# soulslicer/probabilistic-depth

Measured on AMD Instinct MI355X. Metric: depth-volumes/sec (D=64, 256x512), higher is better.
Workload: dtype f32 (fp16-pair products on MFMA, fp32 accumulate)

## Files before the change

### probabilistic-depth_amd/csrc/sweep_dist.hip

```cpp
#include <hip/hip_runtime.h>

#include <atomic>
#include <climits>
#include <cstdlib>

#include "dist_layout.hpp"
#include "epipolar_probe.hpp"
#include "geometry.hpp"
#include "kernels.hpp"
#include "sweep_workspace.hpp"
#include "wave_util.hpp"

#include "sweep_dist_knobs.hpp"

namespace pdepth {

namespace {

using namespace wv;
typedef _Float16 h8 __attribute__((ext_vector_type(8)));
typedef _Float16 h2 __attribute__((ext_vector_type(2)));
typedef int v2i __attribute__((ext_vector_type(2)));

constexpr int DIST_MAXV = 8;

struct DistArgs {
    SweepArgs a;
    const char* packed;
    const float* stats;
    int* queue;
    int* qcnt;
    int qstride;
    int tiles_x, ntile;
    int one_each;
    int nblk;
    int nonce;
};
#define KARG(type, field) kernarg_at<type>(offsetof(DistArgs, field))


__device__ __forceinline__ float dist_exp(float x) {
    return __builtin_amdgcn_exp2f((x < -1000.0f ? -1000.0f : x) * 1.44269502162933349609375f);
}

template <int MAXB, int NAC>
struct __attribute__((aligned(16))) DistLds {
    static constexpr int XSTRIDE = MAXB * 16 + 4;
    float Ys[16 * XSTRIDE];
    float Qs[(MAXB + 3) / 4 * 256 + 8];
    _Float16 Bs[NAC * 4 * 16 * 8];
    float rp[4 * 16 * 2];
    float mus[dist::MAX_C + 8];
    float xf[DIST_MAXV * 12];
    float cst[8];
    float red[4 * 16 * 4];
    float dcl[128];
    int ctab[2][64 * 2];
    int ired[2][2];
    int brow[MAXB + 2];
    v4i rec[2];
    int iflag;
    unsigned char wide[64];
};

template <int NCHK, int NH>
__global__ __launch_bounds__(256, NH == 1 ? DIST_OCC1 : DIST_OCC2) void sweep_dist_kernel(DistArgs da) {
    constexpr int NAC = 2 * NCHK + 1;
    constexpr int MP = NCHK + 1;
    constexpr int MAXB = NH == 1 ? DIST_MAXB1 : DIST_MAXB2;
    constexpr int NC = 4 * NH;
    constexpr int QPL = 8 * NCHK + 3;
    constexpr int NS = NH == 1 ? DIST_SETS1 : DIST_SETS2;
    typedef DistLds<MAXB, NAC> Lds;
    constexpr int XSTRIDE = Lds::XSTRIDE;
    __shared__ Lds L;
#ifdef DIST_STAMPS
    unsigned long long stamp_acc[12] = {0, 0, 0, 0, 0, 0, 0, 0, 0, 0, 0, 0};
    unsigned long long stamp_t = __builtin_amdgcn_s_memtime();
#endif
    if (poison_on_foreign_layout(da.a, da.queue, LAYOUT_DIST16)) return;
    const int tid = threadIdx.x;

    {
        const float* dc = KARG(const float*, a.d_candi);
        const int D = KARG(int, a.D);
        for (int k = tid; k < 64 * NH; k += 256) L.dcl[k] = dc[min(k, D - 1)];
    }
    if (tid < 128) { L.ctab[0][tid] = (tid & 1) ? INT_MIN : INT_MAX; L.ctab[1][tid] = (tid & 1) ? INT_MIN : INT_MAX; }
    if (tid < 64) L.wide[tid] = 1;
    if (tid < 2) { L.ired[tid][0] = INT_MAX; L.ired[tid][1] = INT_MIN; }
    __syncthreads();
    if ((int)(tid >> 2) < min(KARG(int, a.B), 64) && epipolar_probe_is_steep(da.a, tid >> 2, tid & 3)) L.wide[tid >> 2] = 0;

    const int xcd = blockIdx.x & 7;
    if (blockIdx.x == 0 && tid == 0) KARG(int*, queue)[DIST_NONCE_SLOT] = KARG(int, nonce);
    auto band_tiles_of = [&](int q) { const int nt = KARG(int, ntile); return (nt >> 3) + (q < (nt & 7) ? 1 : 0); };
    auto band_first_of = [&](int q) {
        const int nt = KARG(int, ntile), qq = nt >> 3, rr8 = nt & 7;
        return q < rr8 ? q * (qq + 1) : rr8 * (qq + 1) + (q - rr8) * qq;
    };
    auto items_of = [&](int q) { return 4 * band_tiles_of(q) * KARG(int, a.B); };
    int own_done = 0;
    auto steal = [&]() -> int {
        int* qcnt = KARG(int*, qcnt);
        const int qs = KARG(int, qstride);
#pragma unroll 1
        for (int j = 1; j < 8; ++j) {
            const int q = (opaque_s(xcd) + j) & 7, nq = items_of(q);
            if (__hip_atomic_load(&qcnt[q * qs], __ATOMIC_RELAXED, __HIP_MEMORY_SCOPE_AGENT) >= nq) continue;
            const int got = atomicAdd(&qcnt[q * qs], 1);
            if (got < nq) return (q << 28) | got;
        }
        return -1;
    };
    auto resolve = [&](int got) -> int {
        const int n_own = items_of(xcd);
        if (!own_done && got < n_own) return (opaque_s(xcd) << 28) | got;
        own_done = 1;
        return steal();
    };
    auto fdiv = [](int nn, int dd) { return (int)(((float)nn + 0.5f) * __builtin_amdgcn_rcpf((float)dd)); };
    auto decode = [&](int item, int& b_, int& tx_, int& ty_, int& sub_) {
        const int ntile = KARG(int, ntile), tiles_x = KARG(int, tiles_x), H = KARG(int, a.H);
        const int qq = ntile >> 3, rr8 = ntile & 7;
        const bool small_idx = (long long)ntile * 4 * KARG(int, a.B) < (1ll << 22);
        const int tiles_y_ = (H + 3) / 4;
        const int q_ = item >> 28, iq = item & 0x0fffffff, band_tiles = band_tiles_of(q_);
        const int tidx = iq >> 2;
        sub_ = iq & 3;
        b_ = small_idx ? fdiv(tidx, band_tiles) : tidx / band_tiles;
        const int ti = tidx - b_ * band_tiles;
        int tile = band_first_of(q_) + ti;
        if (rr8 == 0 && tiles_y_ % 16 == 0 && tiles_y_ * tiles_x == ntile) {
            const int hb_rows = tiles_y_ / 16, half_tiles = hb_rows * tiles_x;
            const int second = ti >= half_tiles ? 1 : 0, tih = ti - second * half_tiles;
            const int hbi = (q_ < 4) == (second == 0) ? q_ : 8 + q_;
            const int cc = small_idx ? fdiv(tih, hb_rows) : tih / hb_rows, r_ = tih - cc * hb_rows;
            tile = (hbi * hb_rows + r_) * tiles_x + cc;
        } else if (rr8 == 0 && qq % tiles_x == 0) {
            const int band_rows = qq / tiles_x, tc = small_idx ? fdiv(ti, band_rows) : ti / band_rows;
            tile = (q_ * band_rows + (ti - tc * band_rows)) * tiles_x + tc;
        }
        ty_ = small_idx ? fdiv(tile, tiles_x) : tile / tiles_x;
        tx_ = tile - ty_ * tiles_x;
    };
#define ONE_EACH (KARG(int, one_each) != 0)
    __syncthreads();

    int state = 0;
    int n_direct = 0;
    int got_own = (tid == 0 && !ONE_EACH) ? atomicAdd(&KARG(int*, qcnt)[xcd * KARG(int, qstride)], 1) : (int)(blockIdx.x >> 3);
    int next_item = -1;
    auto resolve_next = [&]() { if (opaque_v((int)threadIdx.x) == 0) next_item = ONE_EACH ? -1 : resolve(got_own); };
    constexpr int REC_WIDE = 1, REC_BELOW = 2, REC_FIRST = 4;
    auto publish = [&](int slot, int item) {
        v4i r = v4i{item, 0, 0, 0};
        if (item >= 0) {
            int b, tx, ty, sub;
            decode(item, b, tx, ty, sub);
            const bool wide = b < 64 ? L.wide[b] != 0 : false;
            const int x0 = wide ? tx * 16 : tx * 16 + 8 * (sub & 1), y0 = wide ? ty * 4 + sub : ty * 4 + 2 * (sub >> 1);
            r.y = b;
            r.z = (y0 << 16) | x0;
            r.w = (wide ? REC_WIDE : 0) | (y0 >= KARG(int, a.H) ? REC_BELOW : 0) | ((tx | ty | sub) == 0 ? REC_FIRST : 0);
        }
        L.rec[slot] = r;
    };
    constexpr bool EARLY = DIST_DECODE_EARLY != 0;
    constexpr bool POP_EARLY = EARLY && DIST_PREFETCH == 0;
    auto record_next = [&]() {
        if (opaque_v((int)threadIdx.x) == 0) {
            publish(state & 1, next_item);
            if (POP_EARLY && !ONE_EACH && !own_done) got_own = atomicAdd(&KARG(int*, qcnt)[xcd * KARG(int, qstride)], 1);
        }
    };
    auto publish_next = [&]() {
        if (opaque_v((int)threadIdx.x) == 0) {
            if (!EARLY) publish(state & 1, next_item);
            if (!POP_EARLY && !ONE_EACH && !own_done) got_own = atomicAdd(&KARG(int*, qcnt)[xcd * KARG(int, qstride)], 1);
        }
    };
    constexpr bool PF = DIST_PREFETCH != 0;
    constexpr int ZW = 64 + 128 * NCHK;
    static_assert(4 * ZW + 128 <= (int)(sizeof(Lds::Qs) / sizeof(float)), "the prefetch zone does not fit L.Qs");
    auto dma_pixels = [&](int wave, int b, int p4) {
        const int H = KARG(int, a.H), W = KARG(int, a.W), C = KARG(int, a.C), HW = H * W;
        const int kq = (opaque_v((int)threadIdx.x) & 63) >> 4;
        const __amdgpu_buffer_rsrc_t rray =
            __builtin_amdgcn_make_buffer_rsrc((void*)(KARG(const float*, a.rays) + (size_t)b * 3 * HW), 0, 3 * HW * 4, 0x00020000);
        const __amdgpu_buffer_rsrc_t rref = __builtin_amdgcn_make_buffer_rsrc(
            (void*)(KARG(const float*, a.ref) + (size_t)b * KARG(long long, a.ref_bstride)), 0, C * HW * 4, 0x00020000);
        dma_b32(rray, lds_addr_of(&L.Qs[wave * ZW]), kq < 3 ? kq * HW * 4 + p4 : OOB, 0);
#pragma unroll
        for (int mm = 0; mm < NCHK; ++mm)
#pragma unroll
            for (int j = 0; j < 2; ++j) {
                const int cr = 8 * wave + 4 * j + kq;
                dma_b32(rref, lds_addr_of(&L.Qs[wave * ZW + 64 + 128 * mm + 64 * j]), cr < C - 32 * mm ? cr * HW * 4 + p4 : OOB, 32 * mm * HW * 4);
            }
        if (wave == 0) {
#pragma unroll
            for (int j = 0; j < 2; ++j) {
                const int cr = 4 * j + kq;
                dma_b32(rref, lds_addr_of(&L.Qs[4 * ZW + 64 * j]), cr < C - 32 * NCHK ? cr * HW * 4 + p4 : OOB, 32 * NCHK * HW * 4);
            }
        }
    };
    auto prefetch_next = [&](int wave) {
        const v4i nrec = L.rec[state & 1];
        if (__builtin_amdgcn_readfirstlane(nrec.x) < 0) return;
        const int fl = __builtin_amdgcn_readfirstlane(nrec.w);
        if (fl & REC_BELOW) return;
        const int b = __builtin_amdgcn_readfirstlane(nrec.y), xy = __builtin_amdgcn_readfirstlane(nrec.z);
        const int H = KARG(int, a.H), W = KARG(int, a.W);
        const int n = opaque_v((int)threadIdx.x) & 15;
        const int x = (xy & 0xffff) + ((fl & REC_WIDE) ? n : (n & 7));
        const int y = (xy >> 16) + ((fl & REC_WIDE) ? 0 : (n >> 3));
        dma_pixels(wave, b, (min(y, H - 1) * W + min(x, W - 1)) * 4);
        state |= 4;
    };
    if (tid == 0) {
        publish(0, ONE_EACH ? (got_own < items_of(xcd) ? (xcd << 28) | got_own : -1) : resolve(got_own));
        if (!ONE_EACH && !own_done) got_own = atomicAdd(&KARG(int*, qcnt)[xcd * KARG(int, qstride)], 1);
    }
    PDEPTH_LDS_BARRIER();
#define PDEPTH_POP_WAIT(n) __builtin_amdgcn_s_waitcnt(0x0f70 | (n))
    PDEPTH_POP_WAIT(0);

    for (;;) {
        const v4i rec = L.rec[state & 1];
        state ^= 1;
        const int pf = state & 4;
        state ^= pf;
        if (__builtin_amdgcn_readfirstlane(rec.x) < 0) break;
        DSTAMP(0)
        const int wave = opaque_s(__builtin_amdgcn_readfirstlane((int)threadIdx.x >> 6));
        const int b = __builtin_amdgcn_readfirstlane(rec.y), xy0 = __builtin_amdgcn_readfirstlane(rec.z), recfl = __builtin_amdgcn_readfirstlane(rec.w);
        const int H = KARG(int, a.H), W = KARG(int, a.W), V = KARG(int, a.V), C = KARG(int, a.C), D = KARG(int, a.D);
        const bool wide = (recfl & REC_WIDE) != 0;

        {
            if (recfl & REC_BELOW) {
                resolve_next();
                if (EARLY) record_next();
                publish_next();
                PDEPTH_LDS_BARRIER();
                PDEPTH_POP_WAIT(0);
                continue;
            }
            const int tid = opaque_v((int)threadIdx.x), lane = tid & 63;
            const int n = lane & 15, kq = lane >> 4, tq = wave * 4 + kq;
            const int a32 = (lane ^ 32) << 2;
            const int HW = H * W;
            int p;
            bool xlive;
            float ray[3], rv[MP][2];
            {
                const __amdgpu_buffer_rsrc_t rray =
                    __builtin_amdgcn_make_buffer_rsrc((void*)(KARG(const float*, a.rays) + (size_t)b * 3 * HW), 0, 3 * HW * 4, 0x00020000);
                const __amdgpu_buffer_rsrc_t rref = __builtin_amdgcn_make_buffer_rsrc(
                    (void*)(KARG(const float*, a.ref) + (size_t)b * KARG(long long, a.ref_bstride)), 0, C * HW * 4, 0x00020000);
                const int x = (xy0 & 0xffff) + (wide ? n : (n & 7));
                const int y = (xy0 >> 16) + (wide ? 0 : (n >> 3));
                xlive = x < W && y < H;
                p = min(y, H - 1) * W + min(x, W - 1);
                if (PF) {
                    if (!pf) dma_pixels(wave, b, p * 4);
                } else {
#pragma unroll
                    for (int i = 0; i < 3; ++i) ray[i] = __builtin_bit_cast(float, __builtin_amdgcn_raw_buffer_load_b32(rray, p * 4, i * HW * 4, 0));
#pragma unroll
                    for (int mm = 0; mm < MP; ++mm) {
                        const bool mine = mm < NCHK || wave == 0;
#pragma unroll
                        for (int i = 0; i < 2; ++i)
                            rv[mm][i] = __builtin_bit_cast(float, __builtin_amdgcn_raw_buffer_load_b32(
                                rref, mine && 2 * tq + i < C - 32 * mm ? ((2 * tq + i) * HW + p) * 4 : OOB, 32 * mm * HW * 4, 0));
                    }
                }
            }
            if (EARLY) { resolve_next(); record_next(); }
            DSTAMP(1)
            const bool new_b = b + 1 != state >> 3;
            if (new_b) {
                state = (state & 7) | ((b + 1) << 3);
                const int tid = opaque_v((int)threadIdx.x), lane = tid & 63;
                const float* st = KARG(const float*, stats) + (size_t)b * STATS_STRIDE;
                if (wave == 0) {
                    float am = st[STATS_AMAX + lane], sv = st[STATS_VAR + lane], sl_ = st[STATS_LAG + lane], m2 = st[lane] * st[lane];
                    if (lane + 64 < STATS_VAR) {
                        am = fmaxf(am, st[STATS_AMAX + lane + 64]); sv += st[STATS_VAR + lane + 64]; sl_ += st[STATS_LAG + lane + 64];
                        m2 += st[lane + 64] * st[lane + 64];
                    }
                    float dhi = fabsf(L.dcl[lane]), dlo = -dhi;
                    if (NH == 2) { const float d2 = fabsf(L.dcl[lane + 64]); dhi = fmaxf(dhi, d2); dlo = fmaxf(dlo, -d2); }
                    {
                        const int x32 = (lane ^ 32) << 2;
                        am = fmaxf(am, bperm_f(x32, am)); sv += bperm_f(x32, sv); sl_ += bperm_f(x32, sl_); m2 += bperm_f(x32, m2);
                        dhi = fmaxf(dhi, bperm_f(x32, dhi)); dlo = fmaxf(dlo, bperm_f(x32, dlo));
#define PDEPTH_XOR_STEP(M) { const int pat = ((M) << 10) | 0x1f; \
                             am = fmaxf(am, __builtin_bit_cast(float, __builtin_amdgcn_ds_swizzle(__builtin_bit_cast(int, am), pat))); \
                             sv += __builtin_bit_cast(float, __builtin_amdgcn_ds_swizzle(__builtin_bit_cast(int, sv), pat)); \
                             sl_ += __builtin_bit_cast(float, __builtin_amdgcn_ds_swizzle(__builtin_bit_cast(int, sl_), pat)); \
                             m2 += __builtin_bit_cast(float, __builtin_amdgcn_ds_swizzle(__builtin_bit_cast(int, m2), pat)); \
                             dhi = fmaxf(dhi, __builtin_bit_cast(float, __builtin_amdgcn_ds_swizzle(__builtin_bit_cast(int, dhi), pat))); \
                             dlo = fmaxf(dlo, __builtin_bit_cast(float, __builtin_amdgcn_ds_swizzle(__builtin_bit_cast(int, dlo), pat))); }
                        PDEPTH_XOR_STEP(16) PDEPTH_XOR_STEP(8) PDEPTH_XOR_STEP(4) PDEPTH_XOR_STEP(2) PDEPTH_XOR_STEP(1)
#undef PDEPTH_XOR_STEP
                    }
                    const int e = dist::scale_exponent(am);
                    const float sc = ldexpf(1.0f, e);
                    const float sg = KARG(float, a.sigma);
                    const bool outside = sv > DIST_GUARD_RATIO * sl_ && sv * 10.0f > DIST_GUARD_ENERGY * fabsf(sg);
                    const bool illcond = (float)KARG(int, a.V) * (2.0f * sv + m2) * (dhi + dlo) * 1.1920929e-7f > PDEPTH_COND_LIMIT * fabsf(sg);
                    if (lane == 0) {
                        L.cst[6] = sc; L.cst[7] = ldexpf(refined_rcp(sg), -2 * e);
                        const int pf = reinterpret_cast<const int*>(st + STATS_FLAGS)[0];
                        L.iflag = (pf != 0 ? 1 : 0) | (outside ? 2 : 0) | (illcond ? 4 : 0);
                    }
                    for (int c = lane; c < dist::MAX_C + 8; c += 64) L.mus[c] = st[c] * sc;
                }
                if (tid >= 128 && tid < 128 + V) {
                    const int v = tid - 128;
                    ViewXform xf;
                    make_view_xform(KARG(const float*, a.K) + b * 9, KARG(const float*, a.R) + ((size_t)b * V + v) * 9,
                                    KARG(const float*, a.t) + ((size_t)b * V + v) * 3, KARG(int, a.blas_mode), xf);
    #pragma unroll
                    for (int i = 0; i < 9; ++i) L.xf[v * 12 + i] = xf.kr[i];
    #pragma unroll
                    for (int i = 0; i < 3; ++i) L.xf[v * 12 + 9 + i] = xf.kt[i];
                }
                if (tid == 255) {
                    const float* const cxcy_ = KARG(const float*, a.cxcy);
                    const float cx = cxcy_[b * 2 + 0], cy = cxcy_[b * 2 + 1];
                    L.cst[0] = cx; L.cst[1] = cy; L.cst[2] = refined_rcp(cx); L.cst[3] = refined_rcp(cy);
                    L.cst[4] = (float)W / 2.0f; L.cst[5] = (float)H / 2.0f;
                }
            }
            bool item_ready = !new_b;
            if (KARG(const float*, a.src) != nullptr) {
                if (!item_ready) { PDEPTH_LDS_BARRIER(); item_ready = true; }
                if ((__builtin_amdgcn_readfirstlane(L.iflag) & 7) != 0) {
                    if (opaque_v((int)threadIdx.x) == 0 && (recfl & REC_FIRST)) {
                        reinterpret_cast<int*>(const_cast<float*>(KARG(const float*, stats)) + (size_t)b * STATS_STRIDE + STATS_FLAGS)[1] = 1;
                        n_direct += KARG(int, tiles_x) * (wide ? H : 2 * ((H + 1) >> 1));
                    }
                    if (!EARLY) resolve_next();
                    publish_next();
                    PDEPTH_LDS_BARRIER();
                    PDEPTH_POP_WAIT(0);
                    continue;
                }
            }
            float rr = 0.0f, zc = 0.0f;
            bool centred = false;
            unsigned failmask = 0;
            float cost[NC];
#pragma unroll
            for (int j = 0; j < NC; ++j) cost[j] = 0.0f;
            if (PF) {
                if (pf && (KARG(float*, a.logp_out) != nullptr || KARG(float*, a.depth_out) != nullptr)) {
                    if (NC == 4) asm volatile("s_waitcnt vmcnt(4)" ::: "memory");
                    else asm volatile("s_waitcnt vmcnt(8)" ::: "memory");
                } else {
                    asm volatile("s_waitcnt vmcnt(0)" ::: "memory");
                }
                const float* const z = &L.Qs[wave * ZW];
#pragma unroll
                for (int i = 0; i < 3; ++i) ray[i] = z[16 * i + n];
#pragma unroll
                for (int mm = 0; mm < MP; ++mm)
#pragma unroll
                    for (int i = 0; i < 2; ++i)
                        rv[mm][i] = mm < NCHK ? z[64 + 128 * mm + 16 * (2 * kq + i) + n] : (wave == 0 ? L.Qs[4 * ZW + 16 * (2 * kq + i) + n] : 0.0f);
            }

            constexpr bool RETRY = NH == 2;
            for (int v = 0; v < V; ++v) {
                const char* const srcv_v = RETRY ? nullptr : KARG(const char*, packed) + (size_t)((size_t)b * V + v) * dist::view_bytes(C, H, W);
                const int H_ = H, W_ = W, C_ = C, D_ = D;
#pragma unroll
                for (int h = 0; h < NH; ++h) {
                    if (!item_ready) { PDEPTH_LDS_BARRIER(); item_ready = true; }
                    int attempt = 0;
                    for (;;) {
                    const bool mine = attempt == 0 || (wave >> 1) == attempt - 1;
                    const int H = RETRY ? KARG(int, a.H) : H_, W = RETRY ? KARG(int, a.W) : W_, C = RETRY ? KARG(int, a.C) : C_, D = RETRY ? KARG(int, a.D) : D_;
                    int cell[4];
                    float fw[4], fn[4];
                    {
                        ViewXform xf;
                        {
                            const v4f k0 = *reinterpret_cast<const v4f*>(&L.xf[v * 12]), k1 = *reinterpret_cast<const v4f*>(&L.xf[v * 12 + 4]),
                                      k2 = *reinterpret_cast<const v4f*>(&L.xf[v * 12 + 8]);
                            xf.kr[0] = k0.x; xf.kr[1] = k0.y; xf.kr[2] = k0.z; xf.kr[3] = k0.w; xf.kr[4] = k1.x; xf.kr[5] = k1.y;
                            xf.kr[6] = k1.z; xf.kr[7] = k1.w; xf.kr[8] = k2.x; xf.kt[0] = k2.y; xf.kt[1] = k2.z; xf.kt[2] = k2.w;
                            xf.separate = KARG(int, a.blas_mode);
                        }
                        const v4f c0 = *reinterpret_cast<const v4f*>(&L.cst[0]);
                        const v2f c1 = *reinterpret_cast<const v2f*>(&L.cst[4]);
                        const v4f dk = *reinterpret_cast<const v4f*>(&L.dcl[64 * h + 4 * tq]);
                        float t2a, t2b, t2c;
                        ray_term2(xf, ray[0], ray[1], ray[2], t2a, t2b, t2c);
#pragma unroll
                        for (int j = 0; j < 4; ++j) {
                            const int k = 64 * h + 4 * tq + j;
                            float ix, iy;
                            plane_sample_pos_fast(xf, t2a, t2b, t2c, dk[j], c0.x, c0.y, c0.z, c0.w, c1.x, c1.y, ix, iy);
                            cell[j] = cell_of(ix, iy, W, H, fw[j], fn[j]);
                            if (k >= D || !xlive || !mine) cell[j] = NO_CELL;
                        }
#pragma unroll
                        for (int j = 0; j < 4; ++j) { asm volatile("" : "+v"(fw[j])); asm volatile("" : "+v"(fn[j])); }
                    }
                    DSTAMP(2)
                    if (!centred) {
                        const float sc = L.cst[6], sm2 = -2.0f * sc;
                        float pr = 0.0f, pz = 0.0f;
                        int* const Bw = reinterpret_cast<int*>(L.Bs);
#pragma unroll
                        for (int mm = 0; mm < MP; ++mm) {
                            if (mm == NCHK && wave != 0) continue;
                            const v2f mu2 = *reinterpret_cast<const v2f*>(&L.mus[32 * mm + 2 * tq]);
                            const float x0 = __builtin_fmaf(rv[mm][0], sm2, 2.0f * mu2.x), x1 = __builtin_fmaf(rv[mm][1], sm2, 2.0f * mu2.y);
                            const float s0 = rv[mm][0] * sc, s1 = rv[mm][1] * sc;
                            pr = __builtin_fmaf(x0, x0, pr); pr = __builtin_fmaf(x1, x1, pr);
                            pz = __builtin_fmaf(s0, s0, pz); pz = __builtin_fmaf(s1, s1, pz);
                            const h2 bh = __builtin_convertvector(v2f{x0, x1}, h2);
                            const h2 bl = __builtin_convertvector(v2f{x0 - (float)bh.x, x1 - (float)bh.y}, h2);
                            if (mm < NCHK) {
                                Bw[((mm * 4 + wave) * 16 + n) * 4 + kq] = __builtin_bit_cast(int, bh);
                                Bw[(((NCHK + mm) * 4 + wave) * 16 + n) * 4 + kq] = __builtin_bit_cast(int, bl);
                            } else {
                                Bw[(((2 * NCHK) * 4 + 0) * 16 + n) * 4 + kq] = __builtin_bit_cast(int, bh);
                                Bw[(((2 * NCHK) * 4 + 1) * 16 + n) * 4 + kq] = __builtin_bit_cast(int, bh);
                                Bw[(((2 * NCHK) * 4 + 2) * 16 + n) * 4 + kq] = __builtin_bit_cast(int, bl);
                            }
                        }
                        pr = 0.25f * pr;
                        pr = pr + xor16_f(pr); pr = pr + bperm_f(a32, pr);
                        pz = pz + xor16_f(pz); pz = pz + bperm_f(a32, pz);
                        if (kq == 0) *reinterpret_cast<v2f*>(&L.rp[(wave * 16 + n) * 2]) = v2f{pr, pz};
                    }
                    const int par = (state >> 1) & 1;
                    {
                        int ylo = 32767, yhi = -32768;
                        int rmin = 0, rmax = 0, ry = 0;
                        bool open = false;
#pragma unroll
                        for (int j = 0; j < 4; ++j) {
                            const bool vj = cell[j] != NO_CELL;
                            const int yj = cell_y(cell[j]), xj = cell_x(cell[j]);
                            const bool cont = open && vj && yj == ry;
                            if (open && !cont) {
                                atomicMin(&L.ctab[par][(ry & 63) * 2], rmin);
                                atomicMax(&L.ctab[par][(ry & 63) * 2 + 1], rmax);
                            }
                            rmin = cont ? min(rmin, xj) : xj;
                            rmax = cont ? max(rmax, xj) : xj;
                            ry = yj;
                            open = vj;
                            ylo = min(ylo, vj ? yj : 32767);
                            yhi = max(yhi, yj);
                        }
                        if (open) {
                            atomicMin(&L.ctab[par][(ry & 63) * 2], rmin);
                            atomicMax(&L.ctab[par][(ry & 63) * 2 + 1], rmax);
                        }
                        const int wmin = wave_min_i(ylo), wmax = wave_max_i(yhi);
                        if (lane == 0 && wmin <= wmax) { atomicMin(&L.ired[par][0], wmin); atomicMax(&L.ired[par][1], wmax); }
                    }
                    DSTAMP(3)
                    PDEPTH_LDS_BARRIER();
                    DSTAMP(4)
                    if (!centred) {
#pragma unroll
                        for (int w = 0; w < 4; ++w) {
                            const v2f pp = *reinterpret_cast<const v2f*>(&L.rp[(w * 16 + n) * 2]);
                            rr = rr + pp.x; zc = zc + pp.y;
                        }
                        if (kq == 3) {
                            const dist::Pieces pq = dist::split_pieces(rr < 2.0e9f ? rr : __builtin_nanf(""));
                            h8 sp;
                            sp[0] = (_Float16)dist::PIECE_C1; sp[1] = (_Float16)dist::PIECE_C2; sp[2] = (_Float16)dist::PIECE_C3;
                            sp[3] = pq.p1; sp[4] = pq.p2; sp[5] = pq.p3; sp[6] = (_Float16)0.f; sp[7] = (_Float16)0.f;
                            *reinterpret_cast<h8*>(&L.Bs[(((NAC - 1) * 4 + 3) * 16 + n) * 8]) = sp;
                        }
                        centred = true;
                    }
                    h8 Bv[NAC];
                    const _Float16* const bsl = &L.Bs[(kq * 16 + n) * 8];
#pragma unroll
                    for (int i = 0; i < NAC; ++i) Bv[i] = *reinterpret_cast<const h8*>(bsl + i * 512);
                    const int yb = __builtin_amdgcn_readfirstlane(L.ired[par][0]), yt = __builtin_amdgcn_readfirstlane(L.ired[par][1]);
                    int nb = 0, lo = 0, nblk = 0, fb = 0;
                    bool fits = true;
                    if (yb <= yt) {
                        const int ncell = yt - yb + 1;
                        if (ncell + 1 > 64 || ncell + 1 > MAXB) {
                            fits = false;
                        } else {
                            const v2i e0 = *reinterpret_cast<const v2i*>(&L.ctab[par][((yb + lane) & 63) * 2]);
                            const v2i e1 = *reinterpret_cast<const v2i*>(&L.ctab[par][((yb + lane - 1) & 63) * 2]);
                            const int l0 = min(e0.x, e1.x), h0 = max(e0.y, e1.y);
                            lo = ((l0 + dist::RING) & ~3) - dist::RING;
                            nblk = l0 <= h0 ? (h0 - lo + 2 + 15) >> 4 : 0;
                            const int incl = wave_scan_incl(nblk);
                            nb = __builtin_amdgcn_readlane(incl, 63);
                            fits = nb <= MAXB;
                            fb = incl - nblk;
                        }
                    }
                    const int iflag = __builtin_amdgcn_readfirstlane(L.iflag);
                    if ((iflag & 3) != 0) fits = false;
                    if (DIST_FORCE_DIRECT == -1 || DIST_FORCE_DIRECT == v) fits = false;
                    state ^= 2;
                    const int rowoff = 16 * fb - lo;
                    const bool go = fits && nb > 0;
                    DSTAMP(5)
                    int sl0[4], sl1[4];
                    {
                        constexpr int PB = dist::GROUP_PLANE_BYTES, GB = (8 * NCHK + 4) * PB;
                        const int Wp = dist::wp(W);
                        const int ntex = (n / dist::GROUP) * GB + (n % dist::GROUP) * 16;
                        const char* srcv = RETRY ? KARG(const char*, packed) + (size_t)((size_t)b * KARG(int, a.V) + v) * dist::view_bytes(C, H, W) : srcv_v;
                        const __amdgpu_buffer_rsrc_t rsrc = __builtin_amdgcn_make_buffer_rsrc((void*)srcv, 0, (int)dist::view_bytes(C, H, W), 0x00020000);
                        const int voffA = opaque_v(ntex + kq * PB);
                        h8 S[NS][NAC];
                        int boff = 0;
                        if (go) {
#pragma unroll 1
                            for (int i = 0; i < nblk; ++i) L.brow[fb + i] = lane;
                            const int rho = L.brow[min(lane, MAXB - 1)];
                            const int xs = __builtin_amdgcn_ds_bpermute(4 * rho, lo) + 16 * (lane - __builtin_amdgcn_ds_bpermute(4 * rho, fb));
                            boff = lane < nb ? ((yb + rho + dist::RING) * (Wp / dist::GROUP) + (xs + dist::RING) / dist::GROUP) * GB : OOB;
                        }
                        auto fetch = [&S, rsrc, voffA](int set, int i, int soff) {
                            int voff = voffA;
                            if (i == NAC - 1) {
                                static_assert(PB == 64 && GB % 256 == 0, "kq = bits 6..7 of voffA");
                                asm volatile("" : "+v"(voff));
                                voff -= (int)((0x40800000u >> ((voff >> 3) & 0x18)) & 0xffu);
                            }
                            S[set][i] = __builtin_bit_cast(h8, __builtin_amdgcn_raw_buffer_load_b128(rsrc, voff, soff + i * 4 * PB, 0));
                        };
                        auto fetch_block = [&](int set, int soff) {
#pragma unroll
                            for (int c = 0; c < NCHK; ++c) { fetch(set, c, soff); fetch(set, NCHK + c, soff); }
                            fetch(set, NAC - 1, soff);
                        };
                        const int q = (nb + 3) >> 2, b0 = wave * q, b1 = min(nb, b0 + q);
                        __builtin_amdgcn_s_setprio(1);
                        if (go) {
#pragma unroll
                            for (int u = 0; u < NS; ++u)
                                if (b0 + u < b1) fetch_block(u, __builtin_amdgcn_readlane(boff, b0 + u));
#pragma unroll
                            for (int gq = 0; gq < (MAXB + 15) / 16; ++gq) {
                                const int g = wave + 4 * gq;
                                if (4 * g < nb) {
                                    const int bo = __builtin_amdgcn_ds_bpermute(4 * (4 * g + kq), boff);
                                    const int vq = 4 * g + kq < nb ? bo + ntex : OOB;
                                    dma_b128(rsrc, lds_addr_of(&L.Qs[g * 256]), vq, QPL * PB);
                                }
                            }
                        }
#pragma unroll
                        for (int j = 0; j < 4; ++j) {
                            const bool has = fits && cell[j] != NO_CELL;
                            const int r = has ? cell_y(cell[j]) - yb : 0;
                            const int o0 = __builtin_amdgcn_ds_bpermute(4 * r, rowoff), o1 = __builtin_amdgcn_ds_bpermute(4 * r + 4, rowoff);
                            const int cxx = cell_x(cell[j]);
                            sl0[j] = has ? cxx + o0 : -1;
                            sl1[j] = cxx + o1;
                        }
                        if (go) {
                            auto y_block = [&](int u, int bj, bool more) {
                                const int soff = more ? __builtin_amdgcn_readlane(boff, bj + NS) : 0;
                                v4f acc = v4f{0.f, 0.f, 0.f, 0.f};
#pragma unroll
                                for (int c = 0; c < NCHK; ++c) {
                                    acc = __builtin_amdgcn_mfma_f32_16x16x32_f16(S[u][c], Bv[c], acc, 0, 0, 0);
                                    acc = __builtin_amdgcn_mfma_f32_16x16x32_f16(S[u][c], Bv[NCHK + c], acc, 0, 0, 0);
                                    if (more) fetch(u, c, soff);
                                    acc = __builtin_amdgcn_mfma_f32_16x16x32_f16(S[u][NCHK + c], Bv[c], acc, 0, 0, 0);
                                    if (more) fetch(u, NCHK + c, soff);
                                }
                                acc = __builtin_amdgcn_mfma_f32_16x16x32_f16(S[u][NAC - 1], Bv[NAC - 1], acc, 0, 0, 0);
                                if (more) fetch(u, NAC - 1, soff);
                                int bjo = bj;
                                asm volatile("" : "+s"(bjo));
                                *reinterpret_cast<v4f*>(&L.Ys[n * XSTRIDE + 16 * bjo + 4 * kq]) = acc;
                            };
                            int bi = b0;
#pragma unroll 1
                            for (; bi + 2 * NS <= b1; bi += NS) {
#pragma unroll
                                for (int u = 0; u < NS; ++u) y_block(u, bi + u, true);
                            }
                            if (bi < b1) {
                                if (NS == 1) {
                                    y_block(0, bi, false);
                                } else {
                                    y_block(0, bi, bi + 2 < b1);
                                    if (bi + 1 < b1) y_block(1, bi + 1, false);
                                    if (bi + 2 < b1) y_block(0, bi + 2, false);
                                }
                            }
                            DSTAMP(6)
                            asm volatile("s_waitcnt vmcnt(0)" ::: "memory");
                        }
                        __builtin_amdgcn_s_setprio(0);
                    }
                    DSTAMP(7)
                    PDEPTH_LDS_BARRIER();
                    DSTAMP(8)
                    if (wave == 1) {
                        *reinterpret_cast<v2i*>(&L.ctab[par][lane * 2]) = v2i{INT_MAX, INT_MIN};
                        if (lane == 0) { L.ired[par][0] = INT_MAX; L.ired[par][1] = INT_MIN; }
                    }

                    if (!fits) {
                        if (attempt != 0) failmask |= 1u << ((v * NH + h) * 2 + attempt - 1);
                    } else if (attempt == 0 || (wave >> 1) == attempt - 1) {
                        const float cinv = L.cst[7];
                        const float* yr = &L.Ys[n * XSTRIDE];
#pragma unroll
                        for (int j = 0; j < 4; ++j) {
                            float qv = zc + (fw[j] + fn[j]) * 0.0f;
                            if (sl0[j] >= 0) {
                                const int s0 = sl0[j], s1 = sl1[j];
                                const float Y00 = yr[s0], Y01 = yr[s0 + 1], Y10 = yr[s1], Y11 = yr[s1 + 1];
                                const v4f qa = *reinterpret_cast<const v4f*>(&L.Qs[s0 * 4]);
                                const float dy1 = L.Qs[s0 * 4 + 5];
                                const float ex = 1.0f - fw[j], ey = 1.0f - fn[j];
                                const float w00 = ey * ex, w01 = ey * fw[j], w10 = fn[j] * ex, w11 = fn[j] * fw[j];
                                const float ys = __builtin_fmaf(w11, Y11, __builtin_fmaf(w10, Y10, __builtin_fmaf(w01, Y01, w00 * Y00)));
                                const float qi = __builtin_fmaf(w11, qa.z, __builtin_fmaf(w10, qa.y, w01 * qa.x));
                                const float qo = __builtin_fmaf(w01, dy1, w10 * qa.w);
                                qv = ys - __builtin_fmaf(w11, qo, w00 * qi);
                            }
                            cost[4 * h + j] = cost[4 * h + j] + qv * cinv;
                        }
                    }
                    DSTAMP(9)
                    if (!RETRY) {
                        if (!fits) failmask |= 3u << ((v * NH + h) * 2);
                        break;
                    }
                    if (attempt == 0) {
                        if (fits) break;
                        if ((iflag & 3) != 0 || DIST_FORCE_DIRECT == -1 || DIST_FORCE_DIRECT == v) {
                            failmask |= 3u << ((v * NH + h) * 2);
                            break;
                        }
                    } else if (attempt == 2) {
                        break;
                    }
                    ++attempt;
                    }
                }
            }

            if (failmask != 0) {
                const int H = KARG(int, a.H), W = KARG(int, a.W), V = KARG(int, a.V), C = KARG(int, a.C), D = KARG(int, a.D);
                const int b = opaque_s((state >> 3) - 1);
                const v4f c0 = *reinterpret_cast<const v4f*>(&L.cst[0]), c1 = *reinterpret_cast<const v4f*>(&L.cst[4]);
                const bool ovf = (L.iflag & 1) != 0;
                (void)0;
#pragma unroll 1
                for (int vhh = 0; vhh < V * NH * 2; ++vhh) {
                    if (!(failmask >> vhh & 1u)) continue;
                    if (tid == 0) ++n_direct;
                    if ((wave >> 1) != (vhh & 1)) continue;
                    const int vh = vhh >> 1, v = vh / NH, h = vh - v * NH;
                    ViewXform xf;
#pragma unroll
                    for (int i = 0; i < 9; ++i) xf.kr[i] = L.xf[v * 12 + i];
#pragma unroll
                    for (int i = 0; i < 3; ++i) xf.kt[i] = L.xf[v * 12 + 9 + i];
                    xf.separate = KARG(int, a.blas_mode);
                    float t2a, t2b, t2c;
                    ray_term2(xf, ray[0], ray[1], ray[2], t2a, t2b, t2c);
                    const char* srcv = KARG(const char*, packed) + (size_t)((size_t)b * V + v) * dist::view_bytes(C, H, W);
#pragma unroll 1
                    for (int j = 0; j < 4; ++j) {
                        const int k = 64 * h + 4 * tq + j;
                        float ix, iy, fwj, fnj;
                        plane_sample_pos_fast(xf, t2a, t2b, t2c, L.dcl[k], c0.x, c0.y, c0.z, c0.w, c1.x, c1.y, ix, iy);
                        int cellj = cell_of(ix, iy, W, H, fwj, fnj);
                        if (k >= D || !xlive) cellj = NO_CELL;
                        float qv = zc + (fwj + fnj) * 0.0f;
                        if (cellj != NO_CELL) {
                            const int cxx = cell_x(cellj), cyy = cell_y(cellj);
                            const float ex = 1.0f - fwj, ey = 1.0f - fnj;
                            const float w00 = ey * ex, w01 = ey * fwj, w10 = fnj * ex, w11 = fnj * fwj;
                            const long long t00 = dist::texel_offset(C, H, W, 0, cyy + dist::RING, cxx + dist::RING), t01 = dist::texel_offset(C, H, W, 0, cyy + dist::RING, cxx + dist::RING + 1);
                            const long long t10 = dist::texel_offset(C, H, W, 0, cyy + dist::RING + 1, cxx + dist::RING), t11 = dist::texel_offset(C, H, W, 0, cyy + dist::RING + 1, cxx + dist::RING + 1);
                            const long long pstep = dist::texel_offset(C, H, W, 1, 0, 0);
                            float part = 0.0f;
#pragma unroll 1
                            for (int g = 0; g < 4 * NCHK + 1; ++g) {
                                const bool tail = g == 4 * NCHK;
                                const char* ph = srcv + (tail ? 8 * NCHK : g) * pstep;
                                const char* pl = srcv + (tail ? 8 * NCHK + 1 : 4 * NCHK + g) * pstep;
                                const h8 a00 = *reinterpret_cast<const h8*>(ph + t00), a01 = *reinterpret_cast<const h8*>(ph + t01);
                                const h8 a10 = *reinterpret_cast<const h8*>(ph + t10), a11 = *reinterpret_cast<const h8*>(ph + t11);
                                const h8 l00 = *reinterpret_cast<const h8*>(pl + t00), l01 = *reinterpret_cast<const h8*>(pl + t01);
                                const h8 l10 = *reinterpret_cast<const h8*>(pl + t10), l11 = *reinterpret_cast<const h8*>(pl + t11);
                                const h8 rh = *reinterpret_cast<const h8*>(&L.Bs[(((tail ? 2 * NCHK : (g >> 2)) * 4 + (tail ? 0 : (g & 3))) * 16 + n) * 8]);
                                const h8 rl = *reinterpret_cast<const h8*>(&L.Bs[(((tail ? 2 * NCHK : NCHK + (g >> 2)) * 4 + (tail ? 2 : (g & 3))) * 16 + n) * 8]);
#pragma unroll
                                for (int i = 0; i < 8; ++i) {
                                    float val = ((float)a00[i] + (float)l00[i]) * w00;
                                    val = __builtin_fmaf((float)a01[i] + (float)l01[i], w01, val);
                                    val = __builtin_fmaf((float)a10[i] + (float)l10[i], w10, val);
                                    val = __builtin_fmaf((float)a11[i] + (float)l11[i], w11, val);
                                    const float rq = -0.5f * ((float)rh[i] + (float)rl[i]);
                                    const float diff = val - rq;
                                    part = __builtin_fmaf(diff, diff, part);
                                }
                            }
                            qv = part + (fwj + fnj) * 0.0f;
                        }
                        if (ovf) qv = __builtin_nanf("");
                        const float cj = qv * L.cst[7];
#pragma unroll
                        for (int jj = 0; jj < NC; ++jj) cost[jj] = cost[jj] + (jj == 4 * h + j ? cj : 0.0f);
                    }
                }
            }
            if (!EARLY) resolve_next();
            const int HW4 = KARG(int, a.H) * KARG(int, a.W) * 4;
            const int ovoff = xlive ? 4 * kq * HW4 + p * 4 : OOB;
            const int pl0 = 16 * wave * HW4;
            if (float* const cost_out = KARG(float*, a.cost_out)) {
                const __amdgpu_buffer_rsrc_t rc = __builtin_amdgcn_make_buffer_rsrc((void*)(cost_out + (size_t)b * D * (HW4 >> 2)), 0, D * HW4, 0x00020000);
#pragma unroll
                for (int j = 0; j < NC; ++j)
                    __builtin_amdgcn_raw_buffer_store_b32(__builtin_bit_cast(int, cost[j]), rc, ovoff, pl0 + (64 * (j >> 2) + (j & 3)) * HW4, 0);
            }
            float* const logp_out = KARG(float*, a.logp_out);
            float* const depth_out = KARG(float*, a.depth_out);
            if (logp_out || depth_out) {
                {
                    float mx = -INFINITY;
#pragma unroll
                    for (int j = 0; j < NC; ++j)
                        mx = max_raw(mx, 64 * (j >> 2) + 4 * tq + (j & 3) < D ? cost[j] : -INFINITY);
                    mx = max_raw(mx, xor16_f(mx));
                    mx = max_raw(mx, bperm_f(a32, mx));
                    float ssum = 0.0f, esum = 0.0f;
#pragma unroll
                    for (int j = 0; j < NC; ++j) {
                        const int k = 64 * (j >> 2) + 4 * tq + (j & 3);
                        const float ek = k < D ? dist_exp(cost[j] - mx) : 0.0f;
                        ssum = ssum + ek;
                        esum = __builtin_fmaf(L.dcl[k], ek, esum);
                    }
                    ssum = ssum + xor16_f(ssum); ssum = ssum + bperm_f(a32, ssum);
                    esum = esum + xor16_f(esum); esum = esum + bperm_f(a32, esum);
                    if (kq == 0) *reinterpret_cast<v4f*>(&L.red[(wave * 16 + n) * 4]) = v4f{mx, ssum, esum, 0.0f};
                }
                DSTAMP(10)
                publish_next();
                PDEPTH_LDS_BARRIER();
                {
                    v4f part[4];
#pragma unroll
                    for (int w = 0; w < 4; ++w) part[w] = *reinterpret_cast<const v4f*>(&L.red[(w * 16 + n) * 4]);
                    const float M = max_raw(max_raw(part[0].x, part[1].x), max_raw(part[2].x, part[3].x));
                    float S_ = 0.0f, E = 0.0f;
#pragma unroll
                    for (int w = 0; w < 4; ++w) {
                        const float scw = part[w].x == -INFINITY ? 0.0f : dist_exp(part[w].x - M);
                        S_ = __builtin_fmaf(part[w].y, scw, S_);
                        E = __builtin_fmaf(part[w].z, scw, E);
                    }
                    const float ls = logf(S_);
                    if (PF) { PDEPTH_POP_WAIT(0); prefetch_next(wave); }
                    {
                        const __amdgpu_buffer_rsrc_t rl = __builtin_amdgcn_make_buffer_rsrc(
                            (void*)(logp_out ? logp_out + (size_t)b * D * (HW4 >> 2) : nullptr), 0, logp_out ? D * HW4 : 0, 0x00020000);
#pragma unroll
                        for (int j = 0; j < NC; ++j)
                            __builtin_amdgcn_raw_buffer_store_b32(__builtin_bit_cast(int, (cost[j] - M) - ls), rl, ovoff,
                                                                  pl0 + (64 * (j >> 2) + (j & 3)) * HW4, 0);
                    }
                    if (depth_out && xlive && tq == 0) depth_out[(size_t)b * (HW4 >> 2) + p] = E / S_;
                }
                if (!PF) PDEPTH_POP_WAIT(NC);
            } else {
                publish_next();
                PDEPTH_LDS_BARRIER();
                PDEPTH_POP_WAIT(0);
                if (PF) prefetch_next(wave);
            }
            DSTAMP(11)
        }
    }
#undef PDEPTH_POP_WAIT
#ifdef DIST_STAMPS
    if ((threadIdx.x & 63) == 0)
        for (int i = 0; i < 12; ++i) atomicAdd(reinterpret_cast<unsigned long long*>(KARG(int*, queue) + 8) + i, stamp_acc[i]);
#endif

    if (opaque_v((int)threadIdx.x) == 0) {
        int* queue = KARG(int*, queue);
        const int nonce = KARG(int, nonce);
        if (ONE_EACH) {
            if (n_direct) {
                int old = atomicAdd(&queue[DIST_DIRECT_LAST_SLOT], 0);
                for (;;) {
                    const int nv = (old >> 20) == nonce ? old + n_direct : (nonce << 20) | n_direct;
                    const int seen = atomicCAS(&queue[DIST_DIRECT_LAST_SLOT], old, nv);
                    if (seen == old) break;
                    old = seen;
                }
            }
        } else {
            if (n_direct) atomicAdd(&queue[DIST_DIRECT_SLOT], n_direct);
            const int done = atomicAdd(&queue[DIST_DONE_SLOT], 1);
            if (done == KARG(int, nblk) - 1) {
                const int nd = atomicAdd(&queue[DIST_DIRECT_SLOT], 0);
                for (int q = 0; q < 8; ++q) KARG(int*, qcnt)[q * KARG(int, qstride)] = 0;
                queue[DIST_DONE_SLOT] = 0;
                queue[DIST_DIRECT_SLOT] = 0;
                queue[DIST_DIRECT_LAST_SLOT] = (nonce << 20) | nd;
            }
        }
    }
}

inline int next_nonce() {
    static std::atomic<unsigned> launches{0};
    return (int)(launches.fetch_add(1) % 2047u) + 1;
}

template <int NCHK, int NH>
hipError_t launch_inst(const SweepArgs& a, const SweepWorkspace& ws, int tiles_x, int tiles, hipStream_t stream) {
    auto kern = sweep_dist_kernel<NCHK, NH>;
    static int per_cu[64] = {0};
    int dev = 0;
    if (hipGetDevice(&dev) != hipSuccess || dev < 0 || dev >= 64) dev = 0;
    if (per_cu[dev] == 0) {
        int nbk = 0;
        if (hipOccupancyMaxActiveBlocksPerMultiprocessor(&nbk, kern, 256, 0) != hipSuccess || nbk <= 0) nbk = 2;
        per_cu[dev] = nbk > 5 ? 5 : nbk;
    }
    long long nblk = ((long long)sweep_device_cus() * per_cu[dev] + 7) & ~7ll;
    DistArgs da;
    da.a = a; da.packed = ws.packed; da.stats = ws.stats; da.queue = ws.queue; da.tiles_x = tiles_x; da.ntile = tiles;
    int qs = DIST_QSTRIDE;
    while (qs * 8 > ws.nflags) qs >>= 1;
    da.qcnt = ws.dist_queue_counters();
    da.qstride = qs;
    da.nonce = next_nonce();
    const long long need = 8ll * ((tiles + 7) / 8) * 4 * a.B;
    da.one_each = need <= DIST_ONE_EACH_X * nblk;
    if (da.one_each) nblk = need;
    da.nblk = (int)nblk;
    hipLaunchKernelGGL(kern, dim3((unsigned)nblk), dim3(256), 0, stream, da);
    return hipGetLastError();
}

}

bool sweep_dist_supports(const SweepArgs& a) {
    const long long hw = (long long)a.H * a.W;
    return a.metric == 0 && a.D <= 128 && a.C <= dist::MAX_C && a.V <= DIST_MAXV && a.W <= 32760 && a.H <= 32760 &&
           hw * a.D * 4 < (1ll << 31) && hw * a.C * 4 < (1ll << 31) && dist::view_bytes(a.C, a.H, a.W) < (1ll << 31) && hw * 12 < (1ll << 31);
}

hipError_t launch_sweep_dist(const SweepArgs& a, void* workspace, hipStream_t stream, bool packed_ready) {
    const int tiles_x = (a.W + 15) / 16, tiles_y = (a.H + 3) / 4, tiles = tiles_x * tiles_y;
    const SweepWorkspace ws = SweepWorkspace::of(workspace, a);
    if (!packed_ready) {
        hipError_t e = launch_pack_dist(a, workspace, stream);
        if (e != hipSuccess) return e;
    }
    const int nck = dist::nchk(a.C);
    hipError_t e;
    if (a.D <= 64)
        e = nck == 0 ? launch_inst<0, 1>(a, ws, tiles_x, tiles, stream)
                     : (nck == 1 ? launch_inst<1, 1>(a, ws, tiles_x, tiles, stream) : launch_inst<2, 1>(a, ws, tiles_x, tiles, stream));
    else
        e = nck == 0 ? launch_inst<0, 2>(a, ws, tiles_x, tiles, stream)
                     : (nck == 1 ? launch_inst<1, 2>(a, ws, tiles_x, tiles, stream) : launch_inst<2, 2>(a, ws, tiles_x, tiles, stream));
    if (e != hipSuccess || a.src == nullptr) return e;
    return launch_sweep_direct_items(a, reinterpret_cast<const int*>(ws.stats + STATS_FLAGS) + 1, STATS_STRIDE, stream);
}

}
```

### probabilistic-depth_amd/csrc/sweep_dist_knobs.hpp

```cpp
#pragma once

#ifndef DIST_MAXB1
#define DIST_MAXB1 24
#endif
#ifndef DIST_MAXB2
#define DIST_MAXB2 34
#endif
#ifndef DIST_OCC1
#define DIST_OCC1 4
#endif
#ifndef DIST_OCC2
#define DIST_OCC2 3
#endif
#ifndef DIST_SETS1
#define DIST_SETS1 1
#endif
#ifndef DIST_SETS2
#define DIST_SETS2 2
#endif
#ifndef DIST_QSTRIDE
#define DIST_QSTRIDE 64
#endif
#ifndef DIST_PREFETCH
#define DIST_PREFETCH 0
#endif
#ifndef DIST_DECODE_EARLY
#define DIST_DECODE_EARLY 1
#endif
#ifndef DIST_ONE_EACH_X
#define DIST_ONE_EACH_X 6
#endif
#ifndef DIST_GUARD_RATIO
#define DIST_GUARD_RATIO 1.7f
#endif
#ifndef DIST_GUARD_ENERGY
#define DIST_GUARD_ENERGY 110.0f
#endif
#ifndef DIST_FORCE_DIRECT
#define DIST_FORCE_DIRECT -2
#endif

#ifdef DIST_STAMPS
#define DSTAMP(i) { const unsigned long long t_ = __builtin_amdgcn_s_memtime(); stamp_acc[i] += t_ - stamp_t; stamp_t = t_; }
#elif defined(DIST_MARKS)
#define DSTAMP(i) asm volatile("; MARK " #i ::: "memory");
#else
#define DSTAMP(i)
#endif
```

Baseline: 11160.

## Move work-queue decode to wave 3 and overlap it with gather wait

Queue ownership (atomic pops, item resolve and publish) moves from wave 0 to a configurable wave, 3 by default. Under a new decode mode the next item is resolved and published inside the gather phase, before the vmcnt wait, so the scalar decode latency hides behind outstanding loads. Gather work is rotated across waves so the queue wave gets a different slice. This adds coupling between scheduling and the fetch loop, and the pop now happens only after the wait.

```diff
diff --git a/probabilistic-depth_amd/csrc/sweep_dist.hip b/probabilistic-depth_amd/csrc/sweep_dist.hip
--- a/probabilistic-depth_amd/csrc/sweep_dist.hip
+++ b/probabilistic-depth_amd/csrc/sweep_dist.hip
@@ -80,6 +80,8 @@
 #endif
     if (poison_on_foreign_layout(da.a, da.queue, LAYOUT_DIST16)) return;
     const int tid = threadIdx.x;
+    constexpr int QT = 64 * DIST_QUEUE_WAVE;
+    static_assert(DIST_QUEUE_WAVE >= 0 && DIST_QUEUE_WAVE < 4, "a workgroup has four waves");
 
     {
         const float* dc = KARG(const float*, a.d_candi);
@@ -149,9 +151,9 @@
 
     int state = 0;
     int n_direct = 0;
-    int got_own = (tid == 0 && !ONE_EACH) ? atomicAdd(&KARG(int*, qcnt)[xcd * KARG(int, qstride)], 1) : (int)(blockIdx.x >> 3);
+    int got_own = (tid == QT && !ONE_EACH) ? atomicAdd(&KARG(int*, qcnt)[xcd * KARG(int, qstride)], 1) : (int)(blockIdx.x >> 3);
     int next_item = -1;
-    auto resolve_next = [&]() { if (opaque_v((int)threadIdx.x) == 0) next_item = ONE_EACH ? -1 : resolve(got_own); };
+    auto resolve_next = [&]() { if (opaque_v((int)threadIdx.x) == QT) next_item = ONE_EACH ? -1 : resolve(got_own); };
     constexpr int REC_WIDE = 1, REC_BELOW = 2, REC_FIRST = 4;
     auto publish = [&](int slot, int item) {
         v4i r = v4i{item, 0, 0, 0};
@@ -168,14 +170,14 @@
     };
     constexpr bool EARLY = DIST_DECODE_EARLY != 0;
     constexpr bool POP_EARLY = EARLY && DIST_PREFETCH == 0;
-    auto record_next = [&]() {
-        if (opaque_v((int)threadIdx.x) == 0) {
-            publish(state & 1, next_item);
-            if (POP_EARLY && !ONE_EACH && !own_done) got_own = atomicAdd(&KARG(int*, qcnt)[xcd * KARG(int, qstride)], 1);
+    auto record_next = [&](bool decode = true, bool pop = true) {
+        if (opaque_v((int)threadIdx.x) == QT) {
+            if (decode) publish(state & 1, next_item);
+            if (pop && POP_EARLY && !ONE_EACH && !own_done) got_own = atomicAdd(&KARG(int*, qcnt)[xcd * KARG(int, qstride)], 1);
         }
     };
     auto publish_next = [&]() {
-        if (opaque_v((int)threadIdx.x) == 0) {
+        if (opaque_v((int)threadIdx.x) == QT) {
             if (!EARLY) publish(state & 1, next_item);
             if (!POP_EARLY && !ONE_EACH && !own_done) got_own = atomicAdd(&KARG(int*, qcnt)[xcd * KARG(int, qstride)], 1);
         }
@@ -219,7 +221,7 @@
         dma_pixels(wave, b, (min(y, H - 1) * W + min(x, W - 1)) * 4);
         state |= 4;
     };
-    if (tid == 0) {
+    if (tid == QT) {
         publish(0, ONE_EACH ? (got_own < items_of(xcd) ? (xcd << 28) | got_own : -1) : resolve(got_own));
         if (!ONE_EACH && !own_done) got_own = atomicAdd(&KARG(int*, qcnt)[xcd * KARG(int, qstride)], 1);
     }
@@ -279,7 +281,7 @@
                     }
                 }
             }
-            if (EARLY) { resolve_next(); record_next(); }
+            if (DIST_DECODE_EARLY == 1) { resolve_next(); record_next(); }
             DSTAMP(1)
             const bool new_b = b + 1 != state >> 3;
             if (new_b) {
@@ -341,11 +343,12 @@
             if (KARG(const float*, a.src) != nullptr) {
                 if (!item_ready) { PDEPTH_LDS_BARRIER(); item_ready = true; }
                 if ((__builtin_amdgcn_readfirstlane(L.iflag) & 7) != 0) {
-                    if (opaque_v((int)threadIdx.x) == 0 && (recfl & REC_FIRST)) {
+                    if (opaque_v((int)threadIdx.x) == QT && (recfl & REC_FIRST)) {
                         reinterpret_cast<int*>(const_cast<float*>(KARG(const float*, stats)) + (size_t)b * STATS_STRIDE + STATS_FLAGS)[1] = 1;
                         n_direct += KARG(int, tiles_x) * (wide ? H : 2 * ((H + 1) >> 1));
                     }
-                    if (!EARLY) resolve_next();
+                    if (DIST_DECODE_EARLY != 1) resolve_next();
+                    if (DIST_DECODE_EARLY == 2) record_next();
                     publish_next();
                     PDEPTH_LDS_BARRIER();
                     PDEPTH_POP_WAIT(0);
@@ -549,7 +552,9 @@
                             for (int c = 0; c < NCHK; ++c) { fetch(set, c, soff); fetch(set, NCHK + c, soff); }
                             fetch(set, NAC - 1, soff);
                         };
-                        const int q = (nb + 3) >> 2, b0 = wave * q, b1 = min(nb, b0 + q);
+                        const bool decode_here = DIST_DECODE_EARLY == 2 && v == 0 && h == 0 && attempt == 0;
+                        const int wsh = DIST_DECODE_EARLY == 2 ? (wave + 3 - DIST_QUEUE_WAVE) & 3 : wave;
+                        const int q = (nb + 3) >> 2, b0 = wsh * q, b1 = min(nb, b0 + q);
                         __builtin_amdgcn_s_setprio(1);
                         if (go) {
 #pragma unroll
@@ -608,8 +613,10 @@
                                 }
                             }
                             DSTAMP(6)
-                            asm volatile("s_waitcnt vmcnt(0)" ::: "memory");
-                        }
+                        }
+                        if (decode_here) { resolve_next(); record_next(true, false); }
+                        if (go) asm volatile("s_waitcnt vmcnt(0)" ::: "memory");
+                        if (decode_here) record_next(false, true);
                         __builtin_amdgcn_s_setprio(0);
                     }
                     DSTAMP(7)
@@ -671,7 +678,7 @@
 #pragma unroll 1
                 for (int vhh = 0; vhh < V * NH * 2; ++vhh) {
                     if (!(failmask >> vhh & 1u)) continue;
-                    if (tid == 0) ++n_direct;
+                    if (tid == QT) ++n_direct;
                     if ((wave >> 1) != (vhh & 1)) continue;
                     const int vh = vhh >> 1, v = vh / NH, h = vh - v * NH;
                     ViewXform xf;
@@ -744,16 +751,17 @@
             float* const depth_out = KARG(float*, a.depth_out);
             if (logp_out || depth_out) {
                 {
+                    const int tq4 = opaque_v(4 * tq);
                     float mx = -INFINITY;
 #pragma unroll
                     for (int j = 0; j < NC; ++j)
-                        mx = max_raw(mx, 64 * (j >> 2) + 4 * tq + (j & 3) < D ? cost[j] : -INFINITY);
+                        mx = max_raw(mx, 64 * (j >> 2) + tq4 + (j & 3) < D ? cost[j] : -INFINITY);
                     mx = max_raw(mx, xor16_f(mx));
                     mx = max_raw(mx, bperm_f(a32, mx));
                     float ssum = 0.0f, esum = 0.0f;
 #pragma unroll
                     for (int j = 0; j < NC; ++j) {
-                        const int k = 64 * (j >> 2) + 4 * tq + (j & 3);
+                        const int k = 64 * (j >> 2) + tq4 + (j & 3);
                         const float ek = k < D ? dist_exp(cost[j] - mx) : 0.0f;
                         ssum = ssum + ek;
                         esum = __builtin_fmaf(L.dcl[k], ek, esum);
@@ -801,11 +809,11 @@
     }
 #undef PDEPTH_POP_WAIT
 #ifdef DIST_STAMPS
-    if ((threadIdx.x & 63) == 0)
+    if ((threadIdx.x & 63) == 0 && (DIST_STAMP_WAVE < 0 || (int)(threadIdx.x >> 6) == DIST_STAMP_WAVE))
         for (int i = 0; i < 12; ++i) atomicAdd(reinterpret_cast<unsigned long long*>(KARG(int*, queue) + 8) + i, stamp_acc[i]);
 #endif
 
-    if (opaque_v((int)threadIdx.x) == 0) {
+    if (opaque_v((int)threadIdx.x) == QT) {
         int* queue = KARG(int*, queue);
         const int nonce = KARG(int, nonce);
         if (ONE_EACH) {
diff --git a/probabilistic-depth_amd/csrc/sweep_dist_knobs.hpp b/probabilistic-depth_amd/csrc/sweep_dist_knobs.hpp
--- a/probabilistic-depth_amd/csrc/sweep_dist_knobs.hpp
+++ b/probabilistic-depth_amd/csrc/sweep_dist_knobs.hpp
@@ -25,7 +25,10 @@
 #define DIST_PREFETCH 0
 #endif
 #ifndef DIST_DECODE_EARLY
-#define DIST_DECODE_EARLY 1
+#define DIST_DECODE_EARLY 2
+#endif
+#ifndef DIST_QUEUE_WAVE
+#define DIST_QUEUE_WAVE 3
 #endif
 #ifndef DIST_ONE_EACH_X
 #define DIST_ONE_EACH_X 6
@@ -40,6 +43,9 @@
 #define DIST_FORCE_DIRECT -2
 #endif
 
+#ifndef DIST_STAMP_WAVE
+#define DIST_STAMP_WAVE -1
+#endif
 #ifdef DIST_STAMPS
 #define DSTAMP(i) { const unsigned long long t_ = __builtin_amdgcn_s_memtime(); stamp_acc[i] += t_ - stamp_t; stamp_t = t_; }
 #elif defined(DIST_MARKS)
```

Measured after the change: 11440, median of 6. 1.03x the previous value.
